# michaelnny/muzero

Hardware: NVIDIA B200
Metric: mcts_simulations_per_sec_net_eval_incl (higher is better)
Workload: dtype f64 tree statistics / f32 scores; network fp16 x fp16 -> f32 (tcgen05)

## Files before the change

muzero_b200/csrc/conv.cu:

```cuda
#include "net.cuh"
#include "umma.cuh"
#include <cuda_fp16.h>
#include <cstdlib>

namespace mz {
using namespace umma;

typedef __half act_t;
typedef __half2 act2_t;

constexpr int kConvThreads = 384;
constexpr int kEpiThreads = 256;
constexpr int kTileM = 256;
constexpr int kMaxStages = 6;
constexpr int kPlaneSlack = 64;

constexpr int kMaxLayers = 34;

struct LayerDesc {
  const act_t* in;
  const int32_t* in_index;
  const act_t* w;
  const float* bias;
  const float* tab;
// ... 82 lines not shown
__device__ __forceinline__ int4 pack8_relu(const float* v) {
  return make_int4((int)pack2_relu(v[0], v[1]), (int)pack2_relu(v[2], v[3]), (int)pack2_relu(v[4], v[5]),
                   (int)pack2_relu(v[6], v[7]));
}
__device__ __forceinline__ int4 pack8(const float* v) {
  return make_int4((int)pack2(v[0], v[1]), (int)pack2(v[2], v[3]), (int)pack2(v[4], v[5]), (int)pack2(v[6], v[7]));
}

__device__ __forceinline__ void quad_bar_sync(int quad) {
  switch (quad) {
    case 0: asm volatile("bar.sync 2, 64;" ::: "memory"); break;
    case 1: asm volatile("bar.sync 3, 64;" ::: "memory"); break;
    case 2: asm volatile("bar.sync 4, 64;" ::: "memory"); break;
    default: asm volatile("bar.sync 5, 64;" ::: "memory"); break;
  }
}

__device__ __forceinline__ void st_tile(uint32_t addr, const int4& v) {
  asm volatile("st.shared.v4.b32 [%0], {%1, %2, %3, %4};" ::"r"(addr), "r"(v.x), "r"(v.y), "r"(v.z), "r"(v.w) : "memory");
}

__device__ __constant__ int kTapOrder[9] = {4, 0, 1, 2, 3, 5, 6, 7, 8};

template <int kN, int kRows>
__global__ void __maxnreg__(128) conv3x3_kernel(const __grid_constant__ ConvParams p) {
  constexpr bool kSplitK = (kRows == 128);
  extern __shared__ __align__(1024) unsigned char smem[];
  const int tid = threadIdx.x, warp = tid >> 5, lane = tid & 31;
  const int halo = p.Wp + 1;
  const int TP = p.TP;
  const int chunk_g = p.cg < 8 ? p.cg : 8;
  const int chunks_tap = p.cg / chunk_g;
  const uint32_t stage_bytes = (uint32_t)chunk_g * p.N * 16;
  const uint32_t a_bytes = (uint32_t)p.cg * TP * 16;

  unsigned char* sA = smem;
  unsigned char* sW = smem + (((size_t)2 * a_bytes + 127) & ~(size_t)127);
  const uint32_t kStages = (uint32_t)p.stages;
  uint64_t* bars = reinterpret_cast<uint64_t*>(sW + (size_t)kStages * stage_bytes);
  uint64_t* w_full = bars;
  uint64_t* w_empty = bars + kMaxStages;
  uint64_t* a_full = bars + 2 * kMaxStages;
  uint64_t* mma_done = a_full + 2;
  uint64_t* acc_empty = mma_done + 2;
  uint64_t* a_ready = acc_empty + 2;
  uint32_t* tmem_holder = reinterpret_cast<uint32_t*>(a_ready + 4);
  float* s_bias = reinterpret_cast<float*>(tmem_holder + 4);
  float2* s_mm = reinterpret_cast<float2*>(s_bias + 4 * p.N);
  uint32_t* s_mask = reinterpret_cast<uint32_t*>(s_mm + 2 * 128);

  if (tid == 0) {
    tmem_holder[2] = 0;
    for (uint32_t s = 0; s < kStages; ++s) { mbar_init(&w_full[s], 1); mbar_init(&w_empty[s], kSplitK ? 1 : 2); }
    for (int b = 0; b < 2; ++b) {
      mbar_init(&a_full[b], 1); mbar_init(&mma_done[b], 2); mbar_init(&acc_empty[b], kEpiThreads);
      mbar_init(&a_ready[2 * b], kEpiThreads); mbar_init(&a_ready[2 * b + 1], kEpiThreads);
    }
    fence_mbar_init();
  }
  if (warp == 1) tmem_alloc(tmem_holder, 512);
  tc_fence_before();
  __syncthreads();
  tc_fence_after();
  const uint32_t tmem = *tmem_holder;
  const uint32_t s_res_a = smem_u32(tmem_holder + 2);

  const int G = (int)gridDim.x;
  auto first_tile = [&](int l) { int t0 = ((int)blockIdx.x - l * p.rot) % G; return t0 < 0 ? t0 + G : t0; };
  const bool dbg = p.dbg != nullptr;

  if (warp == 0) {
    if (lane == 0) {
      const int per_tile = 9 * chunks_tap;
      uint32_t it = 0, res_items = 0;
      long long t_wait = 0;
      const long long t_begin = clock64();
      for (int l = 0; l < p.num_layers; ++l) {
        const unsigned char* wl = reinterpret_cast<const unsigned char*>(p.L[l].w);
        for (int tile = first_tile(l); tile < p.num_tiles; tile += G) {
          if (!p.resident && p.flags) {
            const LayerDesc& Lr = p.L[l];
            if (Lr.residual && Lr.res_layer >= 0) {
              const unsigned* f = p.flags + (size_t)Lr.res_layer * p.num_tiles + tile;
              unsigned spins = 0;
              while (ld_acquire(f) == 0u) {
                if (++spins > (1u << 26)) { if (p.err) atomicExch(p.err, 1); break; }
              }
            }
            ++res_items;
            asm volatile("st.release.cta.shared.u32 [%0], %1;" ::"r"(s_res_a), "r"(res_items) : "memory");
          }
          for (int c = 0; c < per_tile; ++c, ++it) {
            const uint32_t s = it % kStages, ph = (it / kStages) & 1;
            const long long tw = dbg ? clock64() : 0;
            mbar_wait(&w_empty[s], ph ^ 1);
            if (dbg) t_wait += clock64() - tw;
            if (p.ablate & 4) { mbar_arrive(&w_full[s]); continue; }
            mbar_arrive_expect_tx(&w_full[s], stage_bytes);
            const int ti = p.khalf ? c % 9 : c / chunks_tap, chs = p.khalf ? c / 9 : c - ti * chunks_tap;
            const int src_stage = kTapOrder[ti] * chunks_tap + chs;
            bulk_g2s(sW + (size_t)s * stage_bytes, wl + (size_t)src_stage * stage_bytes, stage_bytes, &w_full[s]);
          }
        }
      }
      if (dbg) { p.dbg[blockIdx.x * 16 + 0] = clock64() - t_begin; p.dbg[blockIdx.x * 16 + 1] = t_wait; }
    }
  } else if (warp == 1 || warp == 3) {
    const uint32_t mhalf = warp == 1 ? 0u : 1u;
    const uint32_t idesc = instr_desc_f16(128, (uint32_t)p.N);
    const uint64_t a_tmpl = smem_desc(0, (uint32_t)TP * 16, 128);
    const uint64_t b_tmpl = smem_desc(0, (uint32_t)p.N * 16, 128);
    const uint32_t a_hi = (uint32_t)(a_tmpl >> 32), a_lo0 = (uint32_t)a_tmpl;
    const uint32_t b_hi = (uint32_t)(b_tmpl >> 32), b_lo0 = (uint32_t)b_tmpl;
    const uint32_t a_kstep = 2u * (uint32_t)TP, b_kstep = 2u * (uint32_t)p.N;
    const uint32_t sA16 = smem_u32(sA) >> 4, sW16 = smem_u32(sW) >> 4, stage16 = stage_bytes >> 4;
    const int ksteps = chunk_g / 2;
    auto desc64 = [](uint32_t lo, uint32_t hi) { return ((uint64_t)hi << 32) | lo; };
    uint32_t st = 0, st_ph = 0;
    uint32_t b_slot = b_lo0 + sW16;
    const uint32_t b_first = b_slot;
    long long t_acc = 0, t_a = 0, t_a_pos[3] = {0, 0, 0};
    const long long t_begin = clock64();
    int i = 0;
    for (int l = 0; l < p.num_layers; ++l)
    for (int tile = first_tile(l); tile < p.num_tiles; tile += G, ++i) {
      const int buf = i & 1;
      const uint32_t uph = (i >> 1) & 1;
      const int pos_in_layer = (tile - first_tile(l)) / G;
      long long tw = dbg ? clock64() : 0;
      mbar_wait(&acc_empty[buf], uph ^ 1);
      long long tw2 = dbg ? clock64() : 0;
      t_acc += tw2 - tw;
      mbar_wait(&a_full[buf], uph);
      const uint32_t rdy_ph = (uint32_t)(((i >> 1) - (buf == 0 ? 1 : 0)) & 1);
      if (p.resident && i > 0) {
        mbar_wait(&a_ready[2 * buf], rdy_ph);
        if (!p.khalf) mbar_wait(&a_ready[2 * buf + 1], rdy_ph);
      }
      if (dbg) { const long long dt = clock64() - tw2; t_a += dt; t_a_pos[pos_in_layer < 2 ? pos_in_layer : 2] += dt; }
      tc_fence_after();
      const uint32_t a_tile = a_lo0 + sA16 + (uint32_t)buf * (a_bytes >> 4) + (uint32_t)halo + (kSplitK ? 0u : 128u * mhalf);
      const uint32_t dacc = tmem + (uint32_t)(buf * 256) + 128u * mhalf;
      uint32_t acc = 0;
      uint32_t stage_no = 0;
      uint4 eL = make_uint4(0, 0, 0, 0), eR = eL, eT = eL, eB = eL;
      if (p.masked) {
        const uint4* em = reinterpret_cast<const uint4*>(s_mask + (buf * 2 + (kSplitK ? 0 : (int)mhalf)) * 16);
        eL = em[0]; eR = em[1]; eT = em[2]; eB = em[3];
      }
      auto run_stage = [&](uint32_t a_lo, uint32_t m0, uint32_t m1, uint32_t m2, uint32_t m3) {
        if (kSplitK && (stage_no & 1u) != mhalf) {
          ++stage_no;
          ++st; b_slot += stage16;
          if (st == kStages) { st = 0; st_ph ^= 1; b_slot = b_first; }
          return;
        }
        ++stage_no;
        mbar_wait(&w_full[st], st_ph);
        tc_fence_after();
        uint32_t b_lo = b_slot;
        if (ksteps == 4) {
          uint32_t al[4], bl[4];
#pragma unroll
          for (int ks = 0; ks < 4; ++ks) { al[ks] = a_lo + (uint32_t)ks * a_kstep; bl[ks] = b_lo + (uint32_t)ks * b_kstep; }
          mma4_f16_elect_masked(dacc, desc64(al[0], a_hi), desc64(al[1], a_hi), desc64(al[2], a_hi), desc64(al[3], a_hi),
                                desc64(bl[0], b_hi), desc64(bl[1], b_hi), desc64(bl[2], b_hi), desc64(bl[3], b_hi), idesc,
                                acc, m0, m1, m2, m3);
          acc = 1;
        } else {
          for (int ks = 0; ks < ksteps; ++ks) {
            mma_f16_elect_masked(dacc, desc64(a_lo, a_hi), desc64(b_lo, b_hi), idesc, acc, m0, m1, m2, m3);
            acc = 1;
            a_lo += a_kstep;
            b_lo += b_kstep;
          }
        }
        commit_elect(&w_empty[st]);
        ++st; b_slot += stage16;
        if (st == kStages) { st = 0; st_ph ^= 1; b_slot = b_first; }
      };
      const int outer = p.khalf ? 2 : 1;
      for (int ko = 0; ko < outer; ++ko) {
        if (p.khalf && ko == 1 && i > 0) { mbar_wait(&a_ready[2 * buf + 1], rdy_ph); tc_fence_after(); }
        for (int ti = 0; ti < 9; ++ti) {
          const int tap = ti == 0 ? 4 : (ti <= 4 ? ti - 1 : ti);
          const int ky = tap / 3, kx = tap - 3 * ky;
          const uint32_t a_tap = a_tile + (uint32_t)((ky - 1) * p.Wp + (kx - 1));
          const uint32_t m0 = (kx == 0 ? eL.x : 0u) | (kx == 2 ? eR.x : 0u) | (ky == 0 ? eT.x : 0u) | (ky == 2 ? eB.x : 0u);
          const uint32_t m1 = (kx == 0 ? eL.y : 0u) | (kx == 2 ? eR.y : 0u) | (ky == 0 ? eT.y : 0u) | (ky == 2 ? eB.y : 0u);
          const uint32_t m2 = (kx == 0 ? eL.z : 0u) | (kx == 2 ? eR.z : 0u) | (ky == 0 ? eT.z : 0u) | (ky == 2 ? eB.z : 0u);
          const uint32_t m3 = (kx == 0 ? eL.w : 0u) | (kx == 2 ? eR.w : 0u) | (ky == 0 ? eT.w : 0u) | (ky == 2 ? eB.w : 0u);
          if (p.khalf) {
            run_stage(a_tap + (uint32_t)(ko * ksteps) * a_kstep, m0, m1, m2, m3);
          } else {
            for (int ch = 0; ch < chunks_tap; ++ch) run_stage(a_tap + (uint32_t)(ch * ksteps) * a_kstep, m0, m1, m2, m3);
          }
        }
      }
      commit_elect(&mma_done[buf]);
    }
    if (dbg && lane == 0 && warp == 1) {
      long long* d = p.dbg + blockIdx.x * 16;
      d[2] = clock64() - t_begin; d[3] = t_acc; d[4] = t_a; d[6] = i;
      d[12] = t_a_pos[0]; d[13] = t_a_pos[1]; d[14] = t_a_pos[2];
    }
  } else if (warp == 2) {
    const int cg = p.cg;
    long long t_wait = 0, t_dep = 0;
    const long long t_begin = clock64();
    int i = 0, bias_layer = -1;
    for (int l = 0; l < p.num_layers; ++l)
    for (int tile = first_tile(l); tile < p.num_tiles; tile += G, ++i) {
      const LayerDesc& L = p.L[l];
      const int buf = i & 1;
      const int r0 = tile * p.tile_stride - halo, r1 = r0 + kRows + 2 * halo;
      const bool handed_over = p.resident && l > 0;
      long long tw = dbg ? clock64() : 0;
      if (L.dep0 >= 0 && !p.resident) {
        if (lane < 6) {
          const int tt = tile - 1 + lane % 3;
          const int dl = lane < 3 ? L.dep0 : L.dep1;
          if (dl >= 0 && tt >= 0 && tt < p.num_tiles) {
            const unsigned* f = p.flags + (size_t)dl * p.num_tiles + tt;
            unsigned spins = 0;
            while (ld_acquire(f) == 0u) {
              ++spins;
              if ((spins & 0xffffu) == 0 && p.err && *reinterpret_cast<volatile int*>(p.err)) break;
              if (spins > (1u << 26)) { if (p.err) atomicExch(p.err, 1); break; }
            }
          }
        }
        __syncwarp();
        asm volatile("fence.proxy.async;" ::: "memory");
      }
      long long tw2 = dbg ? clock64() : 0;
      t_dep += tw2 - tw;
      if (i >= 2) mbar_wait(&mma_done[buf], (uint32_t)(((i - 2) >> 1) & 1));
      if (dbg) t_wait += clock64() - tw2;
      if (l != bias_layer) {
        for (int c4 = lane; c4 * 4 < kN; c4 += 32)
          *reinterpret_cast<float4*>(s_bias + (l & 3) * kN + c4 * 4) = __ldg(reinterpret_cast<const float4*>(L.bias) + c4);
        bias_layer = l;
      }
      if (p.masked) {
        for (int h = 0; h < kRows / 128; ++h)
          for (int w = 0; w < 4; ++w) {
            const int P = tile * p.tile_stride + h * 128 + w * 32 + lane;
            const int q = P % p.PB, y = q / p.Wp, x = q - y * p.Wp;
            const unsigned mL = __ballot_sync(0xffffffffu, x == 0), mR = __ballot_sync(0xffffffffu, x == p.W - 1);
            const unsigned mT = __ballot_sync(0xffffffffu, y == 0), mB = __ballot_sync(0xffffffffu, y == p.H - 1);
            if (lane == 0) {
              uint32_t* m = s_mask + (buf * 2 + h) * 16;
              m[w] = mL; m[4 + w] = mR; m[8 + w] = mT; m[12 + w] = mB;
            }
          }
      }
      const uint32_t dst0 = smem_u32(sA) + (uint32_t)buf * a_bytes;
      if (handed_over) {
        __syncwarp();
        if (lane == 0) mbar_arrive(&a_full[buf]);
        continue;
      }
      const int lo = p.resident ? tile * p.tile_stride : (r0 > 0 ? r0 : 0);
      int hi = L.in_slots ? p.Ptot : p.plane_rows;
      if (p.resident) { const int e = lo + p.tile_stride; hi = e < p.Ptot ? e : p.Ptot; }
      else hi = r1 < hi ? r1 : hi;
      if (r0 < 0 && !p.resident) {
        const int nz = -r0;
        for (int k = lane; k < nz * cg; k += 32) {
          const int g = k / nz, q = k - g * nz;
          asm volatile("st.shared.v4.b32 [%0], {%1, %1, %1, %1};" ::"r"(dst0 + (uint32_t)(g * TP + q) * 16), "r"(0) : "memory");
        }
        fence_proxy_async();
      }
      __syncwarp();
      if (p.ablate & 2) {
        if (lane == 0) mbar_arrive(&a_full[buf]);
      } else {
        if (lane == 0) mbar_arrive_expect_tx(&a_full[buf], (uint32_t)(hi - lo) * 16u * (uint32_t)cg);
        __syncwarp();
        if (!L.in_slots) {
// ... 8 lines not shown
            const size_t slot = L.in_index ? (size_t)L.in_index[b] : (size_t)b;
            bulk_g2s_u32(dst0 + (uint32_t)(g * TP + (s0 - r0)) * 16,
                         L.in + ((slot * cg + g) * p.PB + (size_t)(s0 - b * p.PB)) * 8, (uint32_t)(s1 - s0) * 16u,
                         &a_full[buf]);
          }
        }
      }
    }
    if (dbg && lane == 0) {
      long long* d = p.dbg + blockIdx.x * 16;
      d[7] = clock64() - t_begin; d[8] = t_wait; d[9] = t_dep;
    }
  } else if (warp >= 4) {
    const int quad = warp & 3, chalf = (warp - 4) >> 2;
    const int et = tid - 128;
    constexpr int NC = kN / 32;
    constexpr int NCW = NC >= 2 ? NC / 2 : 1;
    const bool has_cols = chalf * NCW < NC;
    const size_t PR = (size_t)p.plane_rows;
    long long t_wait = 0;
    const long long t_begin = clock64();
    int k = 0;
    for (int l = 0; l < p.num_layers; ++l)
    for (int tile = first_tile(l); tile < p.num_tiles; tile += G, ++k) {
      const LayerDesc& L = p.L[l];
      const bool norm = (L.out_norm != nullptr) || (L.out_slots != nullptr);
      const int buf = k & 1;
      const float* s_bias_l = s_bias + (l & 3) * kN;
      const bool fast = !norm && L.tab == nullptr && L.out != nullptr;
      const int hand = (p.resident && l + 1 < p.num_layers) ? L.fwd : 0;
      bool lo_done = false;
      const uint32_t next_a = smem_u32(sA) + (uint32_t)(buf ^ 1) * a_bytes + (uint32_t)halo * 16;
      const uint32_t tbase = tmem + ((uint32_t)(quad * 32) << 16) + (uint32_t)(buf * 256);
      if (fast) {
        constexpr int NJ = kRows / 128;
        constexpr int STEPS = NJ * NCW;
        int Pj[2];
        size_t Dj[2];
        bool vj[2], inr[2];
#pragma unroll
        for (int j = 0; j < NJ; ++j) {
          Pj[j] = tile * p.tile_stride + j * 128 + quad * 32 + lane;
          int b = 0, pos = 0; bool hl = true;
          inr[j] = Pj[j] < p.Ptot && j * 128 + quad * 32 + lane < p.tile_stride;
          if (inr[j]) split_pos(Pj[j], p, b, pos, hl);
          vj[j] = !hl;
          Dj[j] = (size_t)Pj[j];
// ... 152 lines not shown
                float v[32];
                chunk(c, v);
#pragma unroll
                for (int e = 0; e < 32; ++e) v[e] = (c * 32 + e < p.n_real) ? (v[e] - mn) * inv : 0.0f;
#pragma unroll
                for (int u = 0; u < 4; ++u) {
                  const int4 o4 = pack8(v + 8 * u);
                  if (on) on[(size_t)(c * 4 + u) * PR] = o4;
                  if (os) os[(size_t)(c * 4 + u) * p.PB] = o4;
                  if (hand == 2) st_tile(next_a + (uint32_t)((c * 4 + u) * TP + j * 128 + quad * 32 + lane) * 16, o4);
                }
              }
            }
          }
        }
      }
      if (hand) {
        fence_proxy_async();
        if (!lo_done) mbar_arrive(&a_ready[2 * (buf ^ 1)]);
        mbar_arrive(&a_ready[2 * (buf ^ 1) + 1]);
      }
      tc_fence_before();
      mbar_arrive(&acc_empty[buf]);
      if (p.flags) {
        asm volatile("bar.sync 1, 256;" ::: "memory");
        if (et == 0) st_release(p.flags + (size_t)l * p.num_tiles + tile, 1u);
      }
    }
    if (dbg && et == 0) {
      long long* d = p.dbg + blockIdx.x * 16;
      d[10] = clock64() - t_begin; d[11] = t_wait;
    }
  }
  tc_fence_before();
  __syncthreads();
  if (warp == 1) tmem_dealloc(tmem, 512);
}

__global__ void pack_obs_kernel(const float* __restrict__ obs, act_t* __restrict__ out, int B, int C, int H,
                                int W, int cpad, int plane_rows, int pad) {
  const int Wp = W + pad, PB = (H + pad) * Wp;
  const size_t rows = (size_t)B * PB, n = rows * (cpad / 8);
  for (size_t i = (size_t)blockIdx.x * blockDim.x + threadIdx.x; i < n; i += (size_t)gridDim.x * blockDim.x) {
    const size_t P = i % rows;
    const int g = (int)(i / rows);
    const int pos = (int)(P % PB), b = (int)(P / PB);
    const int y = pos / Wp, x = pos % Wp;
    float v[8];
#pragma unroll
    for (int e = 0; e < 8; ++e) {
      const int c = g * 8 + e;
      v[e] = (c < C && y < H && x < W) ? obs[(((size_t)b * C + c) * H + y) * W + x] : 0.0f;
      v[e] = fminf(fmaxf(v[e], -65504.0f), 65504.0f);
    }
    reinterpret_cast<int4*>(out)[(size_t)g * plane_rows + P] = pack8(v);
  }
}

__global__ void pack_frames_kernel(const uint8_t* __restrict__ frames, const float* __restrict__ planes,
// ... 321 lines not shown
struct ConvNet : NetImpl {
  mz_net_config cfg;
  Geo lat;
  int C;
  int Creal;
  int A, blocks, max_batch, num_sms;
  bool atari;
  int in_cg;
  ConvLayer rep0, dyn0;
  ConvLayer rep_blocks[64], dyn_blocks[64], pred_blocks[64];
  ConvLayer s2_1, s2_2;
  ConvLayer at_blocks[3][4];
  const float* tab;
  Head h_reward, h_policy, h_value;
  act_t *xobs, *b0, *b1, *b2, *b3, *b4;
  unsigned* flags;
  size_t flags_cap;
  int* err_flag;

  static int tp_of(const Geo& g, int rows = kTileM) { return (rows + 2 * (g.Wp() + 1)) | 1; }
  static int plane_rows_of(const Geo& g, int batch) {
    return (batch * g.PB() + kTileM - 1) / kTileM * kTileM + kPlaneSlack;
  }
  static size_t conv_fixed_smem(const Geo& g, int cg, int n, int rows) {
    const int TP = tp_of(g, rows);
    size_t a = (((size_t)2 * cg * TP * 16) + 127) & ~(size_t)127;
    return a + (2 * kMaxStages + 10) * 8 + 16 + (size_t)4 * n * 4 + 2048 + 256 + 64;
  }
  static int conv_stages(const Geo& g, int cg, int n, int rows) {
    const int chunk_g = cg < 8 ? cg : 8;
    const size_t stage = (size_t)chunk_g * n * 16;
    const size_t fixed = conv_fixed_smem(g, cg, n, rows);
    if (fixed + 2 * stage > 227 * 1024) return 0;
    int s = (int)((227 * 1024 - fixed) / stage);
    static const int cap = getenv("MZ_CONV_MAX_STAGES") ? atoi(getenv("MZ_CONV_MAX_STAGES")) : kMaxStages;
    if (s > cap && cap >= 2) s = cap;
    return s > kMaxStages ? kMaxStages : s;
  }
  static size_t conv_smem(const Geo& g, int cg, int n, int rows) {
    const int chunk_g = cg < 8 ? cg : 8;
    return conv_fixed_smem(g, cg, n, rows) + (size_t)conv_stages(g, cg, n, rows) * chunk_g * n * 16;
  }
  static bool fits(const Geo& g, int cg, int n, int rows) { return conv_stages(g, cg, n, rows) >= 2; }

  ConvParams pend;
  Geo pend_geo{0, 0};
  int pend_cg = 0, pend_batch = 0;
  bool pend_sub = false;
  int pend_prev_first = -1, pend_prev_count = 0;
  const act_t* pend_out_base[kMaxLayers];
  const act_t* pend_norm_base[kMaxLayers];
  int pend_pass[kMaxLayers];

  int add_conv(const ConvLayer& L, const Geo& g, const act_t* in, const int32_t* in_index, bool in_slots, int batch,
               const float* tab_, const int32_t* action, const act_t* residual, act_t* out, act_t* out_norm,
               act_t* out_slots, const int32_t* out_index, cudaStream_t st, bool sub = false) {
    const int np = L.passes();
    const int eff_real = L.n_real < L.n_out ? L.n_real : L.n_pass();
    if (pend.num_layers > 0 && (pend_cg != L.cg || pend_geo.H != g.H || pend_geo.W != g.W || pend_batch != batch ||
                                pend.N != L.n_pass() || pend.n_real != eff_real || pend.tab_groups != L.n_out / 8 ||
                                pend.num_layers + np > kMaxLayers || sub || pend_sub)) {
      int rc = flush(st);
      if (rc) return rc;
    }
// ... 66 lines not shown
        LayerDesc& a = pend.L[i];
        const LayerDesc& b = pend.L[i + 1];
        a.fwd = (b.in_slots == 0 && b.in == a.out && a.out) ? 1 : ((b.in_slots == 0 && b.in == a.out_norm && a.out_norm) ? 2 : 0);
        chain = a.fwd != 0;
      }
      if (chain) {
        const int cand[2] = {128, kTileM};
        for (int ci = 0; ci < 2 && !p.resident; ++ci) {
          const int rr = cand[ci];
          if (force_rows && force_rows != rr) continue;
          if (rr == 128 && cg <= 8) continue;
          if (!fits(g, cg, N, rr)) continue;
          const int bpt = rr / p.PB;
          if (bpt < 1) continue;
          if ((batch + bpt - 1) / bpt > sm_cap0) continue;
          p.resident = 1; rows = rr; p.tile_stride = bpt * p.PB;
          static const bool no_khalf = getenv("MZ_CONV_NO_KHALF") != nullptr;
          p.khalf = (rr == kTileM && cg == 16 && !no_khalf) ? 1 : 0;
        }
      }
    }
    p.num_tiles = p.resident ? (p.Ptot + p.tile_stride - 1) / p.tile_stride : (p.Ptot + rows - 1) / rows;
    p.TP = tp_of(g, rows);
    p.stages = conv_stages(g, cg, N, rows);
    p.err = err_flag;
    if (p.stages < 2) { reset_pending(); set_error("conv tile does not fit shared memory for a %dx%d grid", g.H, g.W); return MZ_EINVAL; }
    const size_t smem = conv_smem(g, cg, N, rows);
    const int sm_cap = (cta_limit > 0 && cta_limit < num_sms) ? cta_limit : num_sms;
    const int grid = p.num_tiles < sm_cap ? p.num_tiles : sm_cap;
    p.rot = nl > 1 ? p.num_tiles % grid : 0;
    p.flags = nullptr;
    if (nl > 1 && !p.resident) {
      if ((size_t)nl * p.num_tiles > flags_cap) { reset_pending(); set_error("internal: flag buffer too small"); return MZ_EINVAL; }
      p.flags = flags;
      cudaError_t e = cudaMemsetAsync(flags, 0, (size_t)nl * p.num_tiles * sizeof(unsigned), st);
      if (e != cudaSuccess) { reset_pending(); set_error("cudaMemsetAsync: %s", cudaGetErrorString(e)); return MZ_ECUDA; }
    }
    p.dbg = nullptr;
    static const int ablate = getenv("MZ_CONV_ABLATE") ? atoi(getenv("MZ_CONV_ABLATE")) : 0;
    p.ablate = ablate;
    static const bool debug = getenv("MZ_CONV_DEBUG") != nullptr;
    if (debug) cudaMalloc(&p.dbg, (size_t)grid * 16 * sizeof(long long));
    prof_mark(kProfConv, st, multi_pass ? (nl + 1) / 2 : nl);
    {
      cudaLaunchConfig_t lc = {};
      lc.gridDim = dim3((unsigned)grid); lc.blockDim = dim3(kConvThreads); lc.dynamicSmemBytes = smem; lc.stream = st;
      cudaLaunchAttribute at[1];
      at[0].id = cudaLaunchAttributeCooperative;
      static const bool noncoop = getenv("MZ_CONV_NONCOOP") != nullptr;
      at[0].val.cooperative = (nl > 1 && !noncoop) ? 1 : 0;
      lc.attrs = at; lc.numAttrs = 1;
      cudaError_t le;
      if (rows == 256) {
        if (N == 128) le = cudaLaunchKernelEx(&lc, conv3x3_kernel<128, 256>, p);
        else if (N == 64) le = cudaLaunchKernelEx(&lc, conv3x3_kernel<64, 256>, p);
        else le = cudaLaunchKernelEx(&lc, conv3x3_kernel<32, 256>, p);
      } else {
        if (N == 128) le = cudaLaunchKernelEx(&lc, conv3x3_kernel<128, 128>, p);
        else if (N == 64) le = cudaLaunchKernelEx(&lc, conv3x3_kernel<64, 128>, p);
        else le = cudaLaunchKernelEx(&lc, conv3x3_kernel<32, 128>, p);
      }
      if (le != cudaSuccess) { reset_pending(); set_error("conv3x3_kernel launch: %s", cudaGetErrorString(le)); cudaGetLastError(); return MZ_ECUDA; }
    }
    prof_mark(-1, st);
    reset_pending();
    MZ_LAUNCH_CHECK("conv3x3_kernel");
    if (debug) {
      cudaDeviceSynchronize();
      std::vector<long long> h((size_t)grid * 16);
      cudaMemcpy(h.data(), p.dbg, h.size() * sizeof(long long), cudaMemcpyDeviceToHost);
      cudaFree(p.dbg);
      double a[16] = {0};
      for (int c = 0; c < grid; ++c) for (int k = 0; k < 16; ++k) a[k] += (double)h[(size_t)c * 16 + k] / grid;
      fprintf(stderr, "[conv dbg] %dx%d cg=%d layers=%d items/cta=%.1f | producer total %.0f wait_empty %.0f | mma total %.0f wait_acc %.0f "
              "wait_a %.0f (1st / 2nd / 3rd tile of a layer: %.0f / %.0f / %.0f) | loader total %.0f wait_mma %.0f wait_dep %.0f | "
              "epilogue total %.0f wait_mma %.0f\n",
              g.H, g.W, cg, nl, a[6], a[0], a[1], a[2], a[3], a[4], a[12], a[13], a[14], a[7], a[8], a[9], a[10], a[11]);
    }
    return MZ_OK;
  }
  HeadsParams pend_heads;
  int num_pend_heads = 0;
  size_t pend_heads_smem = 0;
  void add_head(const Head& h, const act_t* act, int batch, float* dst) {
    HeadParams& p = pend_heads.h[num_pend_heads++];
    p.act = act; p.w1 = h.w1; p.b1 = h.b1; p.w2 = h.w2; p.b2 = h.b2; p.dst = dst;
    p.plane_rows = plane_rows_of(lat, batch);
    p.C = Creal; p.H = lat.H; p.W = lat.W; p.pad = grid_pad(); p.mid = h.mid; p.out = h.out; p.kind = h.kind;
    const size_t smem = ((size_t)h.mid * lat.H * lat.W + h.out) * 4;
    if (smem > pend_heads_smem) pend_heads_smem = smem;
  }
  int launch_heads(int batch, cudaStream_t st) {
    if (num_pend_heads == 0) return MZ_OK;
    if (pending_root) pend_heads.root = *pending_root; else pend_heads.root.enabled = 0;
    prof_mark(kProfHead, st);
    head_kernel<<<dim3(batch, num_pend_heads), 128, pend_heads_smem, st>>>(pend_heads);
// ... 358 lines not shown
  net->reset_pending();
  if ((size_t)(p - (char*)arena) > arena_bytes) {
    set_error("internal: net arena overrun (%zu > %zu)", (size_t)(p - (char*)arena), arena_bytes);
    delete net;
    return MZ_ENOMEM;
  }
  cudaError_t e = cudaDeviceSynchronize();
  if (e != cudaSuccess) { set_error("weight repacking failed: %s", cudaGetErrorString(e)); delete net; return MZ_ECUDA; }
  {
    const int npass = N > 128 ? 128 : N;
    auto ok = [&](const Geo& g, int cg, int n) { return ConvNet::fits(g, cg, n, kTileM) || ConvNet::fits(g, cg, n, 128); };
    bool fit = ok(net->lat, N / 8, npass) && (atari || ok(net->lat, net->in_cg, npass));
    if (atari)
      fit = fit && ok(Geo{c.in_h, c.in_w}, 2, 128) && ok(Geo{c.in_h / 2, c.in_w / 2}, 16, 128) &&
            ok(Geo{c.in_h / 4, c.in_w / 4}, N / 8, npass);
    if (!fit) {
      set_error("conv tile does not fit shared memory (grid too wide)");
      delete net;
      return MZ_EINVAL;
    }
  }
  const int smem_max = 227 * 1024;
  e = cudaFuncSetAttribute(conv3x3_kernel<128, 256>, cudaFuncAttributeMaxDynamicSharedMemorySize, smem_max);
  if (e == cudaSuccess) e = cudaFuncSetAttribute(conv3x3_kernel<64, 256>, cudaFuncAttributeMaxDynamicSharedMemorySize, smem_max);
  if (e == cudaSuccess) e = cudaFuncSetAttribute(conv3x3_kernel<32, 256>, cudaFuncAttributeMaxDynamicSharedMemorySize, smem_max);
  if (e == cudaSuccess) e = cudaFuncSetAttribute(conv3x3_kernel<128, 128>, cudaFuncAttributeMaxDynamicSharedMemorySize, smem_max);
  if (e == cudaSuccess) e = cudaFuncSetAttribute(conv3x3_kernel<64, 128>, cudaFuncAttributeMaxDynamicSharedMemorySize, smem_max);
  if (e == cudaSuccess) e = cudaFuncSetAttribute(conv3x3_kernel<32, 128>, cudaFuncAttributeMaxDynamicSharedMemorySize, smem_max);
  if (e == cudaSuccess) e = cudaFuncSetAttribute(head_kernel, cudaFuncAttributePreferredSharedMemoryCarveout, (int)cudaSharedmemCarveoutMaxShared);
  if (e != cudaSuccess) { set_error("cudaFuncSetAttribute: %s", cudaGetErrorString(e)); delete net; return MZ_ECUDA; }
  *out = net;
  return MZ_OK;
}

}
```

muzero_b200/csrc/umma.cuh:

```cuda
#pragma once
#include <cstdint>
#include <cuda_bf16.h>

namespace mz {
namespace umma {

__device__ __forceinline__ uint32_t smem_u32(const void* p) {
  return static_cast<uint32_t>(__cvta_generic_to_shared(p));
}

__device__ __forceinline__ void mbar_init(uint64_t* bar, uint32_t count) {
  asm volatile("mbarrier.init.shared::cta.b64 [%0], %1;" ::"r"(smem_u32(bar)), "r"(count) : "memory");
}
__device__ __forceinline__ void fence_mbar_init() {
  asm volatile("fence.mbarrier_init.release.cluster;" ::: "memory");
}
__device__ __forceinline__ void mbar_arrive_expect_tx(uint64_t* bar, uint32_t bytes) {
  asm volatile("mbarrier.arrive.expect_tx.shared::cta.b64 _, [%0], %1;" ::"r"(smem_u32(bar)), "r"(bytes) : "memory");
}
__device__ __forceinline__ void mbar_arrive(uint64_t* bar) {
  asm volatile("mbarrier.arrive.shared::cta.b64 _, [%0];" ::"r"(smem_u32(bar)) : "memory");
}
__device__ __forceinline__ bool mbar_try_wait(uint64_t* bar, uint32_t parity) {
  uint32_t ok;
// ... 111 lines not shown
      "{\n\t.reg .pred p, q, t;\n\t"
      "setp.ne.b32 p, %10, 0;\n\t"
      "setp.eq.b32 t, 0, 0;\n\t"
      "elect.sync _|q, 0xffffffff;\n\t"
      "@q tcgen05.mma.cta_group::1.kind::f16 [%0], %1, %5, %9, p;\n\t"
      "@q tcgen05.mma.cta_group::1.kind::f16 [%0], %2, %6, %9, t;\n\t"
      "@q tcgen05.mma.cta_group::1.kind::f16 [%0], %3, %7, %9, t;\n\t"
      "@q tcgen05.mma.cta_group::1.kind::f16 [%0], %4, %8, %9, t;\n\t}"
      ::"r"(d_tmem), "l"(a0), "l"(a1), "l"(a2), "l"(a3), "l"(b0), "l"(b1), "l"(b2), "l"(b3), "r"(idesc), "r"(accumulate)
      : "memory");
}
__device__ __forceinline__ void commit_elect(uint64_t* bar) {
  asm volatile(
      "{\n\t.reg .pred q;\n\t"
      "elect.sync _|q, 0xffffffff;\n\t"
      "@q tcgen05.commit.cta_group::1.mbarrier::arrive::one.shared::cluster.b64 [%0];\n\t}" ::"r"(smem_u32(bar))
      : "memory");
}
__device__ __forceinline__ void commit(uint64_t* bar) {
  asm volatile("tcgen05.commit.cta_group::1.mbarrier::arrive::one.shared::cluster.b64 [%0];" ::"r"(smem_u32(bar))
               : "memory");
}

__device__ __forceinline__ void bulk_g2s(void* smem_dst, const void* gsrc, uint32_t bytes, uint64_t* bar) {
  asm volatile("cp.async.bulk.shared::cluster.global.mbarrier::complete_tx::bytes [%0], [%1], %2, [%3];" ::"r"(
                   smem_u32(smem_dst)),
               "l"(gsrc), "r"(bytes), "r"(smem_u32(bar))
               : "memory");
}

__device__ __forceinline__ void bulk_g2s_u32(uint32_t smem_dst, const void* gsrc, uint32_t bytes, uint64_t* bar) {
  asm volatile("cp.async.bulk.shared::cluster.global.mbarrier::complete_tx::bytes [%0], [%1], %2, [%3];" ::"r"(smem_dst),
               "l"(gsrc), "r"(bytes), "r"(smem_u32(bar))
               : "memory");
}

}
}
```

Measured before the change: 1.460 million.

## Add 2-CTA cluster pair variant of conv kernel using cta_group::2 MMA

Adds a paired-CTA variant of the 3x3 conv kernel for 128-channel, 256-row masked multi-layer launches. Each CTA in a 2-CTA cluster loads half the weight columns, and the leader issues cta_group::2 UMMA with M=256 across both CTAs' tiles. The non-leader relays barrier arrivals to the leader. The aim is to halve per-CTA weight traffic and shared-memory staging, which allows deeper weight pipelines. It adds cluster synchronisation overhead and halves the number of independent scheduling units, which risks imbalance and correctness problems in the barrier protocol.

```diff
diff --git a/muzero_b200/csrc/conv.cu b/muzero_b200/csrc/conv.cu
--- a/muzero_b200/csrc/conv.cu
+++ b/muzero_b200/csrc/conv.cu
@@ -128,16 +128,21 @@
 
 __device__ __constant__ int kTapOrder[9] = {4, 0, 1, 2, 3, 5, 6, 7, 8};
 
-template <int kN, int kRows>
+template <int kN, int kRows, bool kPair = false>
 __global__ void __maxnreg__(128) conv3x3_kernel(const __grid_constant__ ConvParams p) {
   constexpr bool kSplitK = (kRows == 128);
+  constexpr int kBarStages = kPair ? 2 * kMaxStages : kMaxStages;
+  static_assert(!kPair || (kN == 128 && kRows == 256), "pair variant: 256-row tiles, N = 128");
   extern __shared__ __align__(1024) unsigned char smem[];
   const int tid = threadIdx.x, warp = tid >> 5, lane = tid & 31;
+  const uint32_t rank = kPair ? cluster_rank() : 0u;
+  const bool leader = rank == 0;
   const int halo = p.Wp + 1;
   const int TP = p.TP;
   const int chunk_g = p.cg < 8 ? p.cg : 8;
   const int chunks_tap = p.cg / chunk_g;
-  const uint32_t stage_bytes = (uint32_t)chunk_g * p.N * 16;
+  const int n_cta = kPair ? p.N / 2 : p.N;
+  const uint32_t stage_bytes = (uint32_t)chunk_g * n_cta * 16;
   const uint32_t a_bytes = (uint32_t)p.cg * TP * 16;
 
   unsigned char* sA = smem;
@@ -145,8 +150,8 @@
   const uint32_t kStages = (uint32_t)p.stages;
   uint64_t* bars = reinterpret_cast<uint64_t*>(sW + (size_t)kStages * stage_bytes);
   uint64_t* w_full = bars;
-  uint64_t* w_empty = bars + kMaxStages;
-  uint64_t* a_full = bars + 2 * kMaxStages;
+  uint64_t* w_empty = bars + kBarStages;
+  uint64_t* a_full = bars + 2 * kBarStages;
   uint64_t* mma_done = a_full + 2;
   uint64_t* acc_empty = mma_done + 2;
   uint64_t* a_ready = acc_empty + 2;
@@ -156,25 +161,34 @@
   uint32_t* s_mask = reinterpret_cast<uint32_t*>(s_mm + 2 * 128);
 
   if (tid == 0) {
+    const uint32_t relayed = (kPair && leader) ? 1u : 0u;
     tmem_holder[2] = 0;
-    for (uint32_t s = 0; s < kStages; ++s) { mbar_init(&w_full[s], 1); mbar_init(&w_empty[s], kSplitK ? 1 : 2); }
+    for (uint32_t s = 0; s < kStages; ++s) { mbar_init(&w_full[s], 1 + relayed); mbar_init(&w_empty[s], kSplitK ? 1 : 2); }
     for (int b = 0; b < 2; ++b) {
-      mbar_init(&a_full[b], 1); mbar_init(&mma_done[b], 2); mbar_init(&acc_empty[b], kEpiThreads);
+      mbar_init(&a_full[b], 1 + relayed); mbar_init(&mma_done[b], 2); mbar_init(&acc_empty[b], kEpiThreads + relayed);
       mbar_init(&a_ready[2 * b], kEpiThreads); mbar_init(&a_ready[2 * b + 1], kEpiThreads);
     }
     fence_mbar_init();
   }
-  if (warp == 1) tmem_alloc(tmem_holder, 512);
-  tc_fence_before();
-  __syncthreads();
+  if (kPair) {
+    if (warp == 1) tmem_alloc2(tmem_holder, 512);
+    tc_fence_before();
+    cluster_sync();
+  } else {
+    if (warp == 1) tmem_alloc(tmem_holder, 512);
+    tc_fence_before();
+    __syncthreads();
+  }
   tc_fence_after();
   const uint32_t tmem = *tmem_holder;
   const uint32_t s_res_a = smem_u32(tmem_holder + 2);
 
-  const int G = (int)gridDim.x;
-  auto first_tile = [&](int l) { int t0 = ((int)blockIdx.x - l * p.rot) % G; return t0 < 0 ? t0 + G : t0; };
+  const int G = kPair ? (int)gridDim.x / 2 : (int)gridDim.x;
+  const int unit = kPair ? (int)blockIdx.x / 2 : (int)blockIdx.x;
+  const int num_units = kPair ? (p.num_tiles + 1) / 2 : p.num_tiles;
+  auto first_unit = [&](int l) { int t0 = (unit - l * p.rot) % G; return t0 < 0 ? t0 + G : t0; };
+  auto tile_of = [&](int u) { return kPair ? 2 * u + (int)rank : u; };
   const bool dbg = p.dbg != nullptr;
-
   if (warp == 0) {
     if (lane == 0) {
       const int per_tile = 9 * chunks_tap;
@@ -183,10 +197,11 @@
       const long long t_begin = clock64();
       for (int l = 0; l < p.num_layers; ++l) {
         const unsigned char* wl = reinterpret_cast<const unsigned char*>(p.L[l].w);
-        for (int tile = first_tile(l); tile < p.num_tiles; tile += G) {
+        for (int u = first_unit(l); u < num_units; u += G) {
+          const int tile = tile_of(u);
           if (!p.resident && p.flags) {
             const LayerDesc& Lr = p.L[l];
-            if (Lr.residual && Lr.res_layer >= 0) {
+            if (Lr.residual && Lr.res_layer >= 0 && tile < p.num_tiles) {
               const unsigned* f = p.flags + (size_t)Lr.res_layer * p.num_tiles + tile;
               unsigned spins = 0;
               while (ld_acquire(f) == 0u) {
@@ -205,20 +220,49 @@
             mbar_arrive_expect_tx(&w_full[s], stage_bytes);
             const int ti = p.khalf ? c % 9 : c / chunks_tap, chs = p.khalf ? c / 9 : c - ti * chunks_tap;
             const int src_stage = kTapOrder[ti] * chunks_tap + chs;
-            bulk_g2s(sW + (size_t)s * stage_bytes, wl + (size_t)src_stage * stage_bytes, stage_bytes, &w_full[s]);
+            if constexpr (kPair) {
+              const unsigned char* src = wl + ((size_t)src_stage * chunk_g * p.N + rank * (uint32_t)n_cta) * 16;
+              for (int g = 0; g < chunk_g; ++g)
+                bulk_g2s(sW + (size_t)s * stage_bytes + (size_t)g * n_cta * 16, src + (size_t)g * p.N * 16, (uint32_t)n_cta * 16u,
+                         &w_full[s]);
+            } else {
+              bulk_g2s(sW + (size_t)s * stage_bytes, wl + (size_t)src_stage * stage_bytes, stage_bytes, &w_full[s]);
+            }
           }
         }
       }
       if (dbg) { p.dbg[blockIdx.x * 16 + 0] = clock64() - t_begin; p.dbg[blockIdx.x * 16 + 1] = t_wait; }
     }
+  } else if (kPair && !leader && (warp == 1 || warp == 3)) {
+    if (warp == 1 && lane == 0) {
+      const int per_tile = 9 * chunks_tap;
+      uint32_t it = 0;
+      int i = 0;
+      for (int l = 0; l < p.num_layers; ++l)
+        for (int u = first_unit(l); u < num_units; u += G, ++i) {
+          const int buf = i & 1;
+          const uint32_t uph = (i >> 1) & 1;
+          if (i >= 2) {
+            mbar_wait(&acc_empty[buf], uph ^ 1);
+            mbar_arrive_cluster(&acc_empty[buf], 0);
+          }
+          mbar_wait(&a_full[buf], uph);
+          mbar_arrive_cluster(&a_full[buf], 0);
+          for (int c = 0; c < per_tile; ++c, ++it) {
+            const uint32_t s = it % kStages, ph = (it / kStages) & 1;
+            mbar_wait(&w_full[s], ph);
+            mbar_arrive_cluster(&w_full[s], 0);
+          }
+        }
+    }
   } else if (warp == 1 || warp == 3) {
     const uint32_t mhalf = warp == 1 ? 0u : 1u;
-    const uint32_t idesc = instr_desc_f16(128, (uint32_t)p.N);
+    const uint32_t idesc = instr_desc_f16(kPair ? 256 : 128, (uint32_t)p.N);
     const uint64_t a_tmpl = smem_desc(0, (uint32_t)TP * 16, 128);
-    const uint64_t b_tmpl = smem_desc(0, (uint32_t)p.N * 16, 128);
+    const uint64_t b_tmpl = smem_desc(0, (uint32_t)n_cta * 16, 128);
     const uint32_t a_hi = (uint32_t)(a_tmpl >> 32), a_lo0 = (uint32_t)a_tmpl;
     const uint32_t b_hi = (uint32_t)(b_tmpl >> 32), b_lo0 = (uint32_t)b_tmpl;
-    const uint32_t a_kstep = 2u * (uint32_t)TP, b_kstep = 2u * (uint32_t)p.N;
+    const uint32_t a_kstep = 2u * (uint32_t)TP, b_kstep = 2u * (uint32_t)n_cta;
     const uint32_t sA16 = smem_u32(sA) >> 4, sW16 = smem_u32(sW) >> 4, stage16 = stage_bytes >> 4;
     const int ksteps = chunk_g / 2;
     auto desc64 = [](uint32_t lo, uint32_t hi) { return ((uint64_t)hi << 32) | lo; };
@@ -229,10 +273,10 @@
     const long long t_begin = clock64();
     int i = 0;
     for (int l = 0; l < p.num_layers; ++l)
-    for (int tile = first_tile(l); tile < p.num_tiles; tile += G, ++i) {
+    for (int u = first_unit(l); u < num_units; u += G, ++i) {
       const int buf = i & 1;
       const uint32_t uph = (i >> 1) & 1;
-      const int pos_in_layer = (tile - first_tile(l)) / G;
+      const int pos_in_layer = (u - first_unit(l)) / G;
       long long tw = dbg ? clock64() : 0;
       mbar_wait(&acc_empty[buf], uph ^ 1);
       long long tw2 = dbg ? clock64() : 0;
@@ -250,11 +294,13 @@
       uint32_t acc = 0;
       uint32_t stage_no = 0;
       uint4 eL = make_uint4(0, 0, 0, 0), eR = eL, eT = eL, eB = eL;
+      uint4 fL = eL, fR = eL, fT = eL, fB = eL;
       if (p.masked) {
-        const uint4* em = reinterpret_cast<const uint4*>(s_mask + (buf * 2 + (kSplitK ? 0 : (int)mhalf)) * 16);
+        const uint4* em = reinterpret_cast<const uint4*>(s_mask + ((kPair ? buf * 4 : buf * 2) + (kSplitK ? 0 : (int)mhalf)) * 16);
         eL = em[0]; eR = em[1]; eT = em[2]; eB = em[3];
-      }
-      auto run_stage = [&](uint32_t a_lo, uint32_t m0, uint32_t m1, uint32_t m2, uint32_t m3) {
+        if (kPair) { fL = em[8]; fR = em[9]; fT = em[10]; fB = em[11]; }
+      }
+      auto run_stage = [&](uint32_t a_lo, uint32_t m0, uint32_t m1, uint32_t m2, uint32_t m3, const uint4& mp) {
         if (kSplitK && (stage_no & 1u) != mhalf) {
           ++stage_no;
           ++st; b_slot += stage16;
@@ -265,7 +311,16 @@
         mbar_wait(&w_full[st], st_ph);
         tc_fence_after();
         uint32_t b_lo = b_slot;
-        if (ksteps == 4) {
+        if constexpr (kPair) {
+          uint32_t al[4], bl[4];
+#pragma unroll
+          for (int ks = 0; ks < 4; ++ks) { al[ks] = a_lo + (uint32_t)ks * a_kstep; bl[ks] = b_lo + (uint32_t)ks * b_kstep; }
+          mma4_f16_elect_masked2(dacc, desc64(al[0], a_hi), desc64(al[1], a_hi), desc64(al[2], a_hi), desc64(al[3], a_hi),
+                                 desc64(bl[0], b_hi), desc64(bl[1], b_hi), desc64(bl[2], b_hi), desc64(bl[3], b_hi), idesc,
+                                 acc, make_uint4(m0, m1, m2, m3), mp);
+          acc = 1;
+          commit2_elect(&w_empty[st]);
+        } else if (ksteps == 4) {
           uint32_t al[4], bl[4];
 #pragma unroll
           for (int ks = 0; ks < 4; ++ks) { al[ks] = a_lo + (uint32_t)ks * a_kstep; bl[ks] = b_lo + (uint32_t)ks * b_kstep; }
@@ -281,7 +336,7 @@
             b_lo += b_kstep;
           }
         }
-        commit_elect(&w_empty[st]);
+        if constexpr (!kPair) commit_elect(&w_empty[st]);
         ++st; b_slot += stage16;
         if (st == kStages) { st = 0; st_ph ^= 1; b_slot = b_first; }
       };
@@ -296,14 +351,22 @@
           const uint32_t m1 = (kx == 0 ? eL.y : 0u) | (kx == 2 ? eR.y : 0u) | (ky == 0 ? eT.y : 0u) | (ky == 2 ? eB.y : 0u);
           const uint32_t m2 = (kx == 0 ? eL.z : 0u) | (kx == 2 ? eR.z : 0u) | (ky == 0 ? eT.z : 0u) | (ky == 2 ? eB.z : 0u);
           const uint32_t m3 = (kx == 0 ? eL.w : 0u) | (kx == 2 ? eR.w : 0u) | (ky == 0 ? eT.w : 0u) | (ky == 2 ? eB.w : 0u);
+          uint4 mp = make_uint4(0, 0, 0, 0);
+          if (kPair) {
+            auto sel = [&](uint32_t l_, uint32_t r_, uint32_t t_, uint32_t b_) {
+              return (kx == 0 ? l_ : 0u) | (kx == 2 ? r_ : 0u) | (ky == 0 ? t_ : 0u) | (ky == 2 ? b_ : 0u);
+            };
+            mp = make_uint4(sel(fL.x, fR.x, fT.x, fB.x), sel(fL.y, fR.y, fT.y, fB.y), sel(fL.z, fR.z, fT.z, fB.z),
+                            sel(fL.w, fR.w, fT.w, fB.w));
+          }
           if (p.khalf) {
-            run_stage(a_tap + (uint32_t)(ko * ksteps) * a_kstep, m0, m1, m2, m3);
+            run_stage(a_tap + (uint32_t)(ko * ksteps) * a_kstep, m0, m1, m2, m3, mp);
           } else {
-            for (int ch = 0; ch < chunks_tap; ++ch) run_stage(a_tap + (uint32_t)(ch * ksteps) * a_kstep, m0, m1, m2, m3);
+            for (int ch = 0; ch < chunks_tap; ++ch) run_stage(a_tap + (uint32_t)(ch * ksteps) * a_kstep, m0, m1, m2, m3, mp);
           }
         }
       }
-      commit_elect(&mma_done[buf]);
+      if constexpr (kPair) commit2_elect(&mma_done[buf]); else commit_elect(&mma_done[buf]);
     }
     if (dbg && lane == 0 && warp == 1) {
       long long* d = p.dbg + blockIdx.x * 16;
@@ -316,13 +379,15 @@
     const long long t_begin = clock64();
     int i = 0, bias_layer = -1;
     for (int l = 0; l < p.num_layers; ++l)
-    for (int tile = first_tile(l); tile < p.num_tiles; tile += G, ++i) {
+    for (int u = first_unit(l); u < num_units; u += G, ++i) {
+      const int tile = tile_of(u);
       const LayerDesc& L = p.L[l];
       const int buf = i & 1;
       const int r0 = tile * p.tile_stride - halo, r1 = r0 + kRows + 2 * halo;
       const bool handed_over = p.resident && l > 0;
       long long tw = dbg ? clock64() : 0;
-      if (L.dep0 >= 0 && !p.resident) {
+      const bool has_tile = !kPair || tile < p.num_tiles;
+      if (L.dep0 >= 0 && !p.resident && has_tile) {
         if (lane < 6) {
           const int tt = tile - 1 + lane % 3;
           const int dl = lane < 3 ? L.dep0 : L.dep1;
@@ -348,21 +413,22 @@
           *reinterpret_cast<float4*>(s_bias + (l & 3) * kN + c4 * 4) = __ldg(reinterpret_cast<const float4*>(L.bias) + c4);
         bias_layer = l;
       }
-      if (p.masked) {
+      if (p.masked && leader) {
+        for (int pc = 0; pc < (kPair ? 2 : 1); ++pc)
         for (int h = 0; h < kRows / 128; ++h)
           for (int w = 0; w < 4; ++w) {
-            const int P = tile * p.tile_stride + h * 128 + w * 32 + lane;
+            const int P = (tile + pc) * p.tile_stride + h * 128 + w * 32 + lane;
             const int q = P % p.PB, y = q / p.Wp, x = q - y * p.Wp;
             const unsigned mL = __ballot_sync(0xffffffffu, x == 0), mR = __ballot_sync(0xffffffffu, x == p.W - 1);
             const unsigned mT = __ballot_sync(0xffffffffu, y == 0), mB = __ballot_sync(0xffffffffu, y == p.H - 1);
             if (lane == 0) {
-              uint32_t* m = s_mask + (buf * 2 + h) * 16;
+              uint32_t* m = s_mask + ((kPair ? buf * 4 + pc * 2 : buf * 2) + h) * 16;
               m[w] = mL; m[4 + w] = mR; m[8 + w] = mT; m[12 + w] = mB;
             }
           }
       }
       const uint32_t dst0 = smem_u32(sA) + (uint32_t)buf * a_bytes;
-      if (handed_over) {
+      if (handed_over || !has_tile) {
         __syncwarp();
         if (lane == 0) mbar_arrive(&a_full[buf]);
         continue;
@@ -417,7 +483,8 @@
     const long long t_begin = clock64();
     int k = 0;
     for (int l = 0; l < p.num_layers; ++l)
-    for (int tile = first_tile(l); tile < p.num_tiles; tile += G, ++k) {
+    for (int u = first_unit(l); u < num_units; u += G, ++k) {
+      const int tile = tile_of(u);
       const LayerDesc& L = p.L[l];
       const bool norm = (L.out_norm != nullptr) || (L.out_slots != nullptr);
       const int buf = k & 1;
@@ -616,7 +683,7 @@
       }
       tc_fence_before();
       mbar_arrive(&acc_empty[buf]);
-      if (p.flags) {
+      if (p.flags && tile < p.num_tiles) {
         asm volatile("bar.sync 1, 256;" ::: "memory");
         if (et == 0) st_release(p.flags + (size_t)l * p.num_tiles + tile, 1u);
       }
@@ -627,8 +694,13 @@
     }
   }
   tc_fence_before();
-  __syncthreads();
-  if (warp == 1) tmem_dealloc(tmem, 512);
+  if constexpr (kPair) {
+    cluster_sync();
+    if (warp == 1) tmem_dealloc2(tmem, 512);
+  } else {
+    __syncthreads();
+    if (warp == 1) tmem_dealloc(tmem, 512);
+  }
 }
 
 __global__ void pack_obs_kernel(const float* __restrict__ obs, act_t* __restrict__ out, int B, int C, int H,
@@ -996,24 +1068,25 @@
   static int plane_rows_of(const Geo& g, int batch) {
     return (batch * g.PB() + kTileM - 1) / kTileM * kTileM + kPlaneSlack;
   }
-  static size_t conv_fixed_smem(const Geo& g, int cg, int n, int rows) {
+  static size_t conv_fixed_smem(const Geo& g, int cg, int n, int rows, bool pair = false) {
     const int TP = tp_of(g, rows);
     size_t a = (((size_t)2 * cg * TP * 16) + 127) & ~(size_t)127;
-    return a + (2 * kMaxStages + 10) * 8 + 16 + (size_t)4 * n * 4 + 2048 + 256 + 64;
-  }
-  static int conv_stages(const Geo& g, int cg, int n, int rows) {
-    const int chunk_g = cg < 8 ? cg : 8;
-    const size_t stage = (size_t)chunk_g * n * 16;
-    const size_t fixed = conv_fixed_smem(g, cg, n, rows);
+    const int bar_stages = pair ? 2 * kMaxStages : kMaxStages;
+    return a + (2 * bar_stages + 10) * 8 + 16 + (size_t)4 * n * 4 + 2048 + (pair ? 512 : 256) + 64;
+  }
+  static size_t stage_bytes_of(int cg, int n, bool pair) { return (size_t)(cg < 8 ? cg : 8) * (pair ? n / 2 : n) * 16; }
+  static int conv_stages(const Geo& g, int cg, int n, int rows, bool pair = false) {
+    const size_t stage = stage_bytes_of(cg, n, pair);
+    const size_t fixed = conv_fixed_smem(g, cg, n, rows, pair);
     if (fixed + 2 * stage > 227 * 1024) return 0;
     int s = (int)((227 * 1024 - fixed) / stage);
     static const int cap = getenv("MZ_CONV_MAX_STAGES") ? atoi(getenv("MZ_CONV_MAX_STAGES")) : kMaxStages;
-    if (s > cap && cap >= 2) s = cap;
-    return s > kMaxStages ? kMaxStages : s;
-  }
-  static size_t conv_smem(const Geo& g, int cg, int n, int rows) {
-    const int chunk_g = cg < 8 ? cg : 8;
-    return conv_fixed_smem(g, cg, n, rows) + (size_t)conv_stages(g, cg, n, rows) * chunk_g * n * 16;
+    if (s > cap && cap >= 2 && !pair) s = cap;
+    const int max_stages = pair ? 2 * kMaxStages : kMaxStages;
+    return s > max_stages ? max_stages : s;
+  }
+  static size_t conv_smem(const Geo& g, int cg, int n, int rows, bool pair = false) {
+    return conv_fixed_smem(g, cg, n, rows, pair) + (size_t)conv_stages(g, cg, n, rows, pair) * stage_bytes_of(cg, n, pair);
   }
   static bool fits(const Geo& g, int cg, int n, int rows) { return conv_stages(g, cg, n, rows) >= 2; }
 
@@ -1126,13 +1199,20 @@
     }
     p.num_tiles = p.resident ? (p.Ptot + p.tile_stride - 1) / p.tile_stride : (p.Ptot + rows - 1) / rows;
     p.TP = tp_of(g, rows);
-    p.stages = conv_stages(g, cg, N, rows);
+    const int sm_cap = (cta_limit > 0 && cta_limit < num_sms) ? cta_limit : num_sms;
+    const bool pair = p.masked && N == 128 && cg == 16 && rows == kTileM && nl > 1 && !p.resident && !multi_pass &&
+                      sm_cap >= 2 && getenv("MZ_CONV_NO_PAIR") == nullptr;
+    p.stages = conv_stages(g, cg, N, rows, pair);
     p.err = err_flag;
     if (p.stages < 2) { reset_pending(); set_error("conv tile does not fit shared memory for a %dx%d grid", g.H, g.W); return MZ_EINVAL; }
-    const size_t smem = conv_smem(g, cg, N, rows);
-    const int sm_cap = (cta_limit > 0 && cta_limit < num_sms) ? cta_limit : num_sms;
-    const int grid = p.num_tiles < sm_cap ? p.num_tiles : sm_cap;
+    const size_t smem = conv_smem(g, cg, N, rows, pair);
+    int grid = p.num_tiles < sm_cap ? p.num_tiles : sm_cap;
     p.rot = nl > 1 ? p.num_tiles % grid : 0;
+    if (pair) {
+      const int units = (p.num_tiles + 1) / 2, pairs = units < sm_cap / 2 ? units : sm_cap / 2;
+      grid = 2 * pairs;
+      p.rot = units % pairs;
+    }
     p.flags = nullptr;
     if (nl > 1 && !p.resident) {
       if ((size_t)nl * p.num_tiles > flags_cap) { reset_pending(); set_error("internal: flag buffer too small"); return MZ_EINVAL; }
@@ -1144,18 +1224,22 @@
     static const int ablate = getenv("MZ_CONV_ABLATE") ? atoi(getenv("MZ_CONV_ABLATE")) : 0;
     p.ablate = ablate;
     static const bool debug = getenv("MZ_CONV_DEBUG") != nullptr;
-    if (debug) cudaMalloc(&p.dbg, (size_t)grid * 16 * sizeof(long long));
+    if (debug) { cudaMalloc(&p.dbg, (size_t)grid * 16 * sizeof(long long)); cudaMemset(p.dbg, 0, (size_t)grid * 16 * sizeof(long long)); }
     prof_mark(kProfConv, st, multi_pass ? (nl + 1) / 2 : nl);
     {
       cudaLaunchConfig_t lc = {};
       lc.gridDim = dim3((unsigned)grid); lc.blockDim = dim3(kConvThreads); lc.dynamicSmemBytes = smem; lc.stream = st;
-      cudaLaunchAttribute at[1];
+      cudaLaunchAttribute at[2];
       at[0].id = cudaLaunchAttributeCooperative;
       static const bool noncoop = getenv("MZ_CONV_NONCOOP") != nullptr;
       at[0].val.cooperative = (nl > 1 && !noncoop) ? 1 : 0;
-      lc.attrs = at; lc.numAttrs = 1;
+      at[1].id = cudaLaunchAttributeClusterDimension;
+      at[1].val.clusterDim.x = 2; at[1].val.clusterDim.y = 1; at[1].val.clusterDim.z = 1;
+      lc.attrs = at; lc.numAttrs = pair ? 2 : 1;
       cudaError_t le;
-      if (rows == 256) {
+      if (pair) {
+        le = cudaLaunchKernelEx(&lc, conv3x3_kernel<128, 256, true>, p);
+      } else if (rows == 256) {
         if (N == 128) le = cudaLaunchKernelEx(&lc, conv3x3_kernel<128, 256>, p);
         else if (N == 64) le = cudaLaunchKernelEx(&lc, conv3x3_kernel<64, 256>, p);
         else le = cudaLaunchKernelEx(&lc, conv3x3_kernel<32, 256>, p);
@@ -1176,6 +1260,8 @@
       cudaFree(p.dbg);
       double a[16] = {0};
       for (int c = 0; c < grid; ++c) for (int k = 0; k < 16; ++k) a[k] += (double)h[(size_t)c * 16 + k] / grid;
+      if (pair)
+        for (int k : {2, 3, 4, 6, 12, 13, 14}) a[k] *= 2.0;
       fprintf(stderr, "[conv dbg] %dx%d cg=%d layers=%d items/cta=%.1f | producer total %.0f wait_empty %.0f | mma total %.0f wait_acc %.0f "
               "wait_a %.0f (1st / 2nd / 3rd tile of a layer: %.0f / %.0f / %.0f) | loader total %.0f wait_mma %.0f wait_dep %.0f | "
               "epilogue total %.0f wait_mma %.0f\n",
@@ -1580,6 +1666,7 @@
   }
   const int smem_max = 227 * 1024;
   e = cudaFuncSetAttribute(conv3x3_kernel<128, 256>, cudaFuncAttributeMaxDynamicSharedMemorySize, smem_max);
+  if (e == cudaSuccess) e = cudaFuncSetAttribute(conv3x3_kernel<128, 256, true>, cudaFuncAttributeMaxDynamicSharedMemorySize, smem_max);
   if (e == cudaSuccess) e = cudaFuncSetAttribute(conv3x3_kernel<64, 256>, cudaFuncAttributeMaxDynamicSharedMemorySize, smem_max);
   if (e == cudaSuccess) e = cudaFuncSetAttribute(conv3x3_kernel<32, 256>, cudaFuncAttributeMaxDynamicSharedMemorySize, smem_max);
   if (e == cudaSuccess) e = cudaFuncSetAttribute(conv3x3_kernel<128, 128>, cudaFuncAttributeMaxDynamicSharedMemorySize, smem_max);
diff --git a/muzero_b200/csrc/umma.cuh b/muzero_b200/csrc/umma.cuh
--- a/muzero_b200/csrc/umma.cuh
+++ b/muzero_b200/csrc/umma.cuh
@@ -157,6 +157,55 @@
                : "memory");
 }
 
+__device__ __forceinline__ uint32_t cluster_rank() {
+  uint32_t r;
+  asm volatile("mov.u32 %0, %%cluster_ctarank;" : "=r"(r));
+  return r;
+}
+__device__ __forceinline__ void cluster_sync() {
+  asm volatile("barrier.cluster.arrive.release.aligned;\n\tbarrier.cluster.wait.acquire.aligned;" ::: "memory");
+}
+__device__ __forceinline__ void mbar_arrive_cluster(uint64_t* bar, uint32_t rank) {
+  asm volatile(
+      "{\n\t.reg .b32 ra;\n\t"
+      "mapa.shared::cluster.u32 ra, %0, %1;\n\t"
+      "mbarrier.arrive.shared::cluster.b64 _, [ra];\n\t}" ::"r"(smem_u32(bar)), "r"(rank)
+      : "memory");
+}
+__device__ __forceinline__ void tmem_alloc2(uint32_t* smem_dst, uint32_t ncols) {
+  asm volatile("tcgen05.alloc.cta_group::2.sync.aligned.shared::cta.b32 [%0], %1;" ::"r"(smem_u32(smem_dst)),
+               "r"(ncols)
+               : "memory");
+  asm volatile("tcgen05.relinquish_alloc_permit.cta_group::2.sync.aligned;" ::: "memory");
+}
+__device__ __forceinline__ void tmem_dealloc2(uint32_t taddr, uint32_t ncols) {
+  asm volatile("tcgen05.dealloc.cta_group::2.sync.aligned.b32 %0, %1;" ::"r"(taddr), "r"(ncols) : "memory");
+}
+__device__ __forceinline__ void mma4_f16_elect_masked2(uint32_t d_tmem, uint64_t a0, uint64_t a1, uint64_t a2, uint64_t a3,
+                                                       uint64_t b0, uint64_t b1, uint64_t b2, uint64_t b3, uint32_t idesc,
+                                                       uint32_t accumulate, const uint4& lo, const uint4& hi) {
+  asm volatile(
+      "{\n\t.reg .pred p, q, t;\n\t"
+      "setp.ne.b32 p, %10, 0;\n\t"
+      "setp.eq.b32 t, 0, 0;\n\t"
+      "elect.sync _|q, 0xffffffff;\n\t"
+      "@q tcgen05.mma.cta_group::2.kind::f16 [%0], %1, %5, %9, {%11, %12, %13, %14, %15, %16, %17, %18}, p;\n\t"
+      "@q tcgen05.mma.cta_group::2.kind::f16 [%0], %2, %6, %9, {%11, %12, %13, %14, %15, %16, %17, %18}, t;\n\t"
+      "@q tcgen05.mma.cta_group::2.kind::f16 [%0], %3, %7, %9, {%11, %12, %13, %14, %15, %16, %17, %18}, t;\n\t"
+      "@q tcgen05.mma.cta_group::2.kind::f16 [%0], %4, %8, %9, {%11, %12, %13, %14, %15, %16, %17, %18}, t;\n\t}"
+      ::"r"(d_tmem), "l"(a0), "l"(a1), "l"(a2), "l"(a3), "l"(b0), "l"(b1), "l"(b2), "l"(b3), "r"(idesc),
+        "r"(accumulate), "r"(lo.x), "r"(lo.y), "r"(lo.z), "r"(lo.w), "r"(hi.x), "r"(hi.y), "r"(hi.z), "r"(hi.w)
+      : "memory");
+}
+__device__ __forceinline__ void commit2_elect(uint64_t* bar) {
+  asm volatile(
+      "{\n\t.reg .pred q;\n\t"
+      "elect.sync _|q, 0xffffffff;\n\t"
+      "@q tcgen05.commit.cta_group::2.mbarrier::arrive::one.shared::cluster.multicast::cluster.b64 [%0], %1;\n\t}"
+      ::"r"(smem_u32(bar)), "h"((uint16_t)3)
+      : "memory");
+}
+
 __device__ __forceinline__ void bulk_g2s(void* smem_dst, const void* gsrc, uint32_t bytes, uint64_t* bar) {
   asm volatile("cp.async.bulk.shared::cluster.global.mbarrier::complete_tx::bytes [%0], [%1], %2, [%3];" ::"r"(
                    smem_u32(smem_dst)),
```

New measurement: 840,500, median of 6. 42.4% lower.
